# yharby/flac-raster

Hardware: AMD Instinct MI355X
Metric: raster MPixels/sec encoded at -c 5 + size ratio vs libFLAC, 1/2/4/8 GPU (higher is better)
Workload: dtype u16->i16 (int32 analysis, exact integer autocorrelation on i8 MFMA)

## Files before the change

### flac-raster_amd/csrc/fra_analyze_w.hip

```cpp
#include <type_traits>

#include "fra_device.h"

namespace fra {

namespace {

constexpr int kWChunks = kMaxBlock / kChunk;
constexpr int kWIters = kWChunks / 64;

struct WaveSmem {
  uint32_t sw[8 * kWChunks];
  double acf[3][9];
};
constexpr uint32_t kBufWords = 8 * kWChunks;

__device__ __forceinline__ int sdw(int t, int d) { return 8 * t + d; }
__device__ __forceinline__ int32_t wsample(const uint32_t* sw, int s) {
  const uint32_t v = sw[sdw(s >> 4, (s & 15) >> 1)];
  return (s & 1) ? hi16(v) : lo16(v);
}
__device__ __forceinline__ void wsync() {
  __builtin_amdgcn_wave_barrier();
  asm volatile("" ::: "memory");
}
constexpr int kWIterDw = 8 * 64;
constexpr int kWinW = 3;
__device__ __forceinline__ uint4 lds4(const uint32_t* p) { return *reinterpret_cast<const uint4*>(p); }
__device__ __forceinline__ void wread_d14(const uint32_t* sw, int lane, int j, uint32_t (&D)[14]) {
  const uint32_t* po = sw + 8 * lane + kWIterDw * j;
  const bool first = j == 0 && lane == 0;
  const uint32_t* pp = first ? po : po - 8;
  const uint4 p0 = lds4(pp), p1 = lds4(pp + 4), o0 = lds4(po), o1 = lds4(po + 4);
  D[0] = first ? 0u : p0.z; D[1] = first ? 0u : p0.w;
  D[2] = first ? 0u : p1.x; D[3] = first ? 0u : p1.y; D[4] = first ? 0u : p1.z; D[5] = first ? 0u : p1.w;
  D[6] = o0.x; D[7] = o0.y; D[8] = o0.z; D[9] = o0.w;
  D[10] = o1.x; D[11] = o1.y; D[12] = o1.z; D[13] = o1.w;
}
__device__ __forceinline__ void unpack28(const uint32_t (&D)[14], int32_t (&x)[28]) {
#pragma unroll
  for (int k = 0; k < 14; k++) {
    x[2 * k] = lo16(D[k]);
    x[2 * k + 1] = hi16(D[k]);
  }
}
__device__ __forceinline__ uint32_t group_sum32(uint32_t v, int ls) {
  if (ls > 0) v = up_add32<0>(v);
  if (ls > 1) v = up_add32<1>(v);
  if (ls > 2) v = up_add32<2>(v);
  if (ls > 3) v = up_add32<3>(v);
  if (ls > 4) v = up_add32<4>(v);
  if (ls > 5) v = up_add32<5>(v);
  return v;
}
__device__ __forceinline__ uint64_t group_sum64(uint64_t v, int ls) {
  if (ls > 0) v = up_add64<0>(v);
  if (ls > 1) v = up_add64<1>(v);
  if (ls > 2) v = up_add64<2>(v);
  if (ls > 3) v = up_add64<3>(v);
  if (ls > 4) v = up_add64<4>(v);
  if (ls > 5) v = up_add64<5>(v);
  return v;
}
__device__ __forceinline__ uint64_t group_sum_auto(uint64_t v, int ls) {
  if (__all(v < (1ull << (32 - ls)))) return group_sum32((uint32_t)v, ls);
  return group_sum64(v, ls);
}
__device__ __forceinline__ double rdlane_f64(double v, int l) {
  const uint64_t b = (uint64_t)__double_as_longlong(v);
  const uint32_t lo = (uint32_t)__builtin_amdgcn_readlane((int)(uint32_t)b, l);
  const uint32_t hi = (uint32_t)__builtin_amdgcn_readlane((int)(uint32_t)(b >> 32), l);
  return __longlong_as_double((long long)(((uint64_t)hi << 32) | lo));
}


template <int MAXLAG>
__device__ inline int levinson_keep(const double (&ac)[MAXLAG + 1], int max_order, double& e, double (&lp)[MAXLAG],
                                    int lo) {
  double lpc[MAXLAG];
#pragma unroll
  for (int j = 0; j < MAXLAG; j++) { lpc[j] = 0.0; lp[j] = 0.0; }
  e = 0.0;
  double err = ac[0];
  int result = max_order;
  bool done = false;
#pragma unroll
  for (int i = 0; i < MAXLAG; i++) {
    if (!done && i < max_order) {
      double r = -ac[i + 1];
#pragma unroll
      for (int j = 0; j < i; j++) r = r - lpc[j] * ac[i - j];
      r = r / err;
      lpc[i] = r;
#pragma unroll
      for (int j = 0; j < (i >> 1); j++) {
        const double tmp = lpc[j];
        lpc[j] = lpc[j] + r * lpc[i - 1 - j];
        lpc[i - 1 - j] = lpc[i - 1 - j] + r * tmp;
      }
      if (i & 1) lpc[i >> 1] = lpc[i >> 1] + lpc[i >> 1] * r;
      err = err * (1.0 - r * r);
      const bool mine = lo == i + 1;
#pragma unroll
      for (int j = 0; j <= i; j++) lp[j] = mine ? -lpc[j] : lp[j];
      e = (mine || (i == 0 && lo == 0)) ? err : e;
      if (!(err > 0.0)) {
        result = (err == 0.0) ? i + 1 : i;
        done = true;
      }
    }
  }
  return result;
}

__device__ __forceinline__ void fixed_guess2_w(const uint32_t (&ps)[5], int P, int lane, int& g1, int& g2,
                                               uint64_t& t1, uint64_t& t2) {
  uint64_t T[5];
  bool small = true;
  uint32_t pv[5];
#pragma unroll
  for (int k = 0; k < 5; k++) {
    pv[k] = lane < (1 << P) ? ps[k] : 0u;
    small = small && pv[k] < (1u << 25);
  }
  if (__all(small)) {
#pragma unroll
    for (int k = 0; k < 5; k++) T[k] = wave_sum32(pv[k]);
  } else {
#pragma unroll
    for (int k = 0; k < 5; k++) {
      uint64_t v = pv[k];
      v = up_add64<0>(v); v = up_add64<1>(v); v = up_add64<2>(v);
      v = up_add64<3>(v); v = up_add64<4>(v); v = up_add64<5>(v);
      T[k] = ((uint64_t)(uint32_t)__builtin_amdgcn_readlane((int)(uint32_t)(v >> 32), 63) << 32) |
             (uint32_t)__builtin_amdgcn_readlane((int)(uint32_t)v, 63);
    }
  }
  int h1 = -1, h2 = -1;
  uint64_t b1 = 0, b2 = 0;
#pragma unroll
  for (int k = 0; k < 5; k++) {
    const bool lt1 = h1 < 0 || T[k] < b1;
    const bool lt2 = !lt1 && (h2 < 0 || T[k] < b2);
    b2 = lt1 ? b1 : (lt2 ? T[k] : b2);
    h2 = lt1 ? h1 : (lt2 ? k : h2);
    b1 = lt1 ? T[k] : b1;
    h1 = lt1 ? k : h1;
  }
  g1 = __builtin_amdgcn_readfirstlane(h1);
  g2 = __builtin_amdgcn_readfirstlane(h2);
  t1 = b1;
  t2 = b2;
}

#ifndef FRA_W_ARITH
#define FRA_W_ARITH 0
#endif
struct WNorm {
  double two_mn, range, rcp;
  uint32_t flip;
};
template <typename T>
__device__ __forceinline__ int32_t wnorm(uint32_t r, const WNorm& q) {
  const int32_t v = (int32_t)((r ^ q.flip) - q.flip);
  const double t = fma((double)v, 2.0, q.two_mn);
  const double q0 = t * q.rcp;
  const double rr = fma(-q0, q.range, t);
  double u = fma(rr, q.rcp, q0);
  u = u - 1.0;
  u = u * 32767.0;
  return (int32_t)u;
}
template <typename T>
__device__ __forceinline__ void wload_lut(const void* base, const WaveDev& wd, int c,
                                          const int32_t* lut, uint32_t* sw, int lane, uint32_t& orv, int32_t& vmin,
                                          int32_t& vmax, bool stamp, const WNorm& wn) {
  constexpr int V = 8 / (int)sizeof(T);
  constexpr int NV = kMaxBlock / 64 / V;
  constexpr uint32_t step = 64 * V;
  using VT = VecT<T, V>;
  const uint32_t w = wd.width;
  const char* b0 = (const char*)((const T*)base + wd.off0 + (int64_t)c * wd.band_stride);
  const uint32_t rsb = wd.row_stride * (uint32_t)sizeof(T);
  const uint32_t qs = step / w, rs = step - qs * w, rstep = qs * rsb;
  uint32_t col = wd.col0 + (uint32_t)lane * V;
  uint32_t roff = 0;
  if (col >= w) {
    const uint32_t q = col / w;
    col -= q * w;
    roff = q * rsb;
  }
  VT x[NV];
#pragma unroll
  for (int kv = 0; kv < NV; kv++) {
    x[kv] = *(const VT*)(b0 + (roff + col * (uint32_t)sizeof(T)));
    col += rs;
    roff += rstep;
    if (col >= w) { col -= w; roff += rsb; }
  }
  if (stamp) FRA_WSTAMP_WAIT(11)
  uint32_t orp = 0;
  i16x2 pmin = {32767, 32767}, pmax = {-32768, -32768};
#pragma unroll
  for (int kv = 0; kv < NV; kv++) {
    int32_t g[V];
    const bool arith = FRA_W_ARITH == 1 || (FRA_W_ARITH == 2 && (kv & 1));
    const uint2 xw = __builtin_bit_cast(uint2, x[kv]);
#pragma unroll
    for (int e = 0; e < V; e++) {
      constexpr int EB = 8 * (int)sizeof(T);
      const uint32_t wsrc = e < V / 2 ? xw.x : xw.y;
      const uint32_t raw = (wsrc >> (EB * (e % (V / 2)))) & ((1u << EB) - 1u);
      g[e] = arith ? wnorm<T>(raw, wn) : *(const int32_t*)((const char*)lut + (raw << 2));
    }
    const int i = (lane + 64 * kv) * V;
#pragma unroll
    for (int h = 0; h < V / 4; h++) {
      const int s = i + 4 * h;
      const uint32_t p0 = __builtin_amdgcn_perm((uint32_t)g[4 * h + 1], (uint32_t)g[4 * h], 0x05040100u);
      const uint32_t p1 = __builtin_amdgcn_perm((uint32_t)g[4 * h + 3], (uint32_t)g[4 * h + 2], 0x05040100u);
      *reinterpret_cast<uint2*>(&sw[sdw(s >> 4, (s & 15) >> 1)]) = make_uint2(p0, p1);
      orp |= p0 | p1;
      const i16x2 a0 = __builtin_bit_cast(i16x2, p0), a1 = __builtin_bit_cast(i16x2, p1);
      pmin = __builtin_elementwise_min(pmin, __builtin_elementwise_min(a0, a1));
      pmax = __builtin_elementwise_max(pmax, __builtin_elementwise_max(a0, a1));
    }
  }
  orv |= (orp | (orp >> 16)) & 0xFFFFu;
  vmin = min(vmin, min((int32_t)pmin.x, (int32_t)pmin.y));
  vmax = max(vmax, max((int32_t)pmax.x, (int32_t)pmax.y));
  if (stamp) FRA_WSTAMP_WAIT(12)
}

template <int O>
__device__ __forceinline__ uint32_t lpc_abs16_w(const uint32_t (&D)[14], const int32_t* q, int sh, bool head) {
  constexpr int NP = (O + 1) / 2;
  fra_short2 Q[NP];
  q_pairs_rev<NP>(q, Q);
  uint32_t acc = 0;
#pragma unroll
  for (int jj = 0; jj < kChunk; jj++) {
    const int32_t r = sample_at(D, 12 + jj) - (pred_raw<NP>(D, 12 + jj, Q) >> sh);
    const uint32_t rb = (uint32_t)r ^ kBias;
    acc = sad_acc(rb, (jj < O && head) ? rb : kBias, acc);
  }
  return acc;
}

template <int O, bool K17>
__device__ __forceinline__ uint32_t lpc_abs16_pk(const uint32_t (&D)[14], const int32_t* q, int sh, bool head,
                                                 uint32_t (&pk)[kChunk / 2], uint32_t& um, uint32_t& hb) {
  constexpr int NP = (O + 1) / 2;
  fra_short2 Q[NP];
  q_pairs_rev<NP>(q, Q);
  uint32_t acc = 0;
  uint32_t u[kChunk];
  hb = 0;
#pragma unroll
  for (int jj = 0; jj < kChunk; jj++) {
    const int32_t r = sample_at(D, 12 + jj) - (pred_raw<NP>(D, 12 + jj, Q) >> sh);
    const uint32_t rb = (uint32_t)r ^ kBias;
    const bool warm = jj < O && head;
    acc = sad_acc(rb, warm ? rb : kBias, acc);
    u[jj] = warm ? 0u : zz32(r);
    um |= u[jj];
  }
#pragma unroll
  for (int p = 0; p < kChunk / 2; p++) pk[p] = (u[2 * p + 1] << 16) | (u[2 * p] & 0xFFFFu);
  if (K17 && __any(um > 0xFFFFu)) {
#pragma unroll
    for (int jj = 0; jj < kChunk; jj++) hb |= (u[jj] >> 16) << jj;
  }
  return acc;
}

}


template <int MAXLAG, int PCAP, bool K17>
#ifndef FRA_W_WAVES
#define FRA_W_WAVES 4
#endif
#ifndef FRA_W_ACF_ITERS
#define FRA_W_ACF_ITERS 4
#endif
#ifndef FRA_W_VGPR_FLOOR
#define FRA_W_VGPR_FLOOR 1
#endif
#ifndef FRA_W_WAVES_MAX
#define FRA_W_WAVES_MAX 8
#endif
__global__ void __launch_bounds__(64) __attribute__((amdgpu_waves_per_eu(FRA_W_WAVES, FRA_W_WAVES_MAX)))
k_analyze_w(JobArgs a, int src) {
  static_assert(MAXLAG == 8 && PCAP >= 4 && PCAP <= 6, "levels 3-6");
  __shared__ WaveSmem S;
  uint32_t* const sw = S.sw;
  const int lane = (int)threadIdx.x;
#if FRA_W_VGPR_FLOOR
  asm volatile("" ::: "v103");
#endif
  FRA_WSTAMP(0)
#ifndef FRA_W_XCD
#define FRA_W_XCD 1
#endif
  int bx = (int)blockIdx.x;
  if (FRA_W_XCD) {
    const int nx = (int)gridDim.x, n8 = nx & ~7;
    const int lin = bx + (int)blockIdx.y * nx;
    if ((nx & 7) == 0 && bx < n8) bx = (lin & 7) * (n8 >> 3) + (bx >> 3);
  }
  const int g = a.frame_base + bx;
  const int c = (int)blockIdx.y;
  const WaveDev wd = a.wave[g];
  if (c >= wd.nch) return;
  FRA_WSTAMP_WAIT(10)
  if (wd.n != kMaxBlock) return;
  constexpr int n = kMaxBlock;
  const int bps = wd.bps;
  const LevelCfg cfg = level_cfg(a.level);
  SfDesc* d = &a.sf[(size_t)g * a.cmax + c];
  uint32_t* const slot = a.tmp + ((size_t)g * a.cmax + c) * a.tmp_stride;
#ifdef FRA_WSTOP
  if (lane == 0) {
    d->type = 1; d->order = 0; d->wasted = 0; d->sbps = (uint8_t)bps; d->cval = 0; d->porder = 0;
    d->method = 0; d->precision = 0; d->shift = 0; d->bits = 8u + (uint32_t)n * (uint32_t)bps;
  }
#endif

  uint32_t orv = 0;
  int32_t vmin = INT32_MAX, vmax = INT32_MIN;
  const void* const raster = a.raster;
  const int32_t* const lut = a.lut + (int64_t)wd.stream * a.lut_stride;
  WNorm wn{};
  if (FRA_W_ARITH) {
    const NormParams np = norm_params(a.streams[wd.stream], a.norm[wd.stream]);
    wn.two_mn = -2.0 * np.mn;
    wn.range = np.range;
    wn.rcp = np.rcp;
    wn.flip = src == ST_I16 ? 0x8000u : (src == ST_I8 ? 0x80u : 0u);
  }
  auto load_samples = [&](uint32_t& ov, int32_t& mn, int32_t& mx, bool first) {
    if (src == ST_U8 || src == ST_I8) wload_lut<uint8_t>(raster, wd, c, lut, sw, lane, ov, mn, mx, first, wn);
    else wload_lut<uint16_t>(raster, wd, c, lut, sw, lane, ov, mn, mx, first, wn);
  };
  load_samples(orv, vmin, vmax, true);
  orv = wave_or32(orv);
  wsync();
  FRA_WSTAMP(1)
  vmin = (int32_t)(wave_min32((uint32_t)vmin ^ 0x80000000u) ^ 0x80000000u);
  vmax = (int32_t)(~wave_min32(~((uint32_t)vmax ^ 0x80000000u)) ^ 0x80000000u);
  FRA_WSTOP_AT(1, orv ^ (uint32_t)vmin ^ (uint32_t)vmax ^ sw[lane] ^ sw[2047 - lane])

  if (vmin == vmax) {
    if (lane == 0) {
      d->type = 0; d->order = 0; d->wasted = 0; d->sbps = (uint8_t)bps; d->cval = vmin;
      d->bits = 8u + (uint32_t)bps; d->porder = 0; d->method = 0; d->precision = 0; d->shift = 0;
      const uint64_t v = (uint64_t)(uint32_t)vmin & ((1ull << bps) - 1);
      const uint64_t blob = v << (64 - 8 - bps);
      slot[0] = (uint32_t)(blob >> 32);
      slot[1] = (uint32_t)blob;
    }
    return;
  }
  const int w = __builtin_ctz(orv);
  const int sbps = bps - w;
  auto shift_wasted = [&]() {
    for (int k = lane; k < (int)kBufWords; k += 64) {
      const uint32_t v = sw[k];
      const uint32_t lo = (uint32_t)(lo16(v) >> w) & 0xFFFFu, hi = (uint32_t)(hi16(v) >> w);
      sw[k] = lo | (hi << 16);
    }
  };
  if (w) shift_wasted();
  wsync();
  const uint32_t hdr = 8u + (uint32_t)w;
  const uint32_t verb = hdr + (uint32_t)n * (uint32_t)sbps;
  constexpr int P = PCAP;
  constexpr int gsl = 8 - P;
  const int prec = qlp_precision(bps, n);
  const int lmax = cfg.max_lpc;

  constexpr int npl = 6 - gsl;
  const int pj = lane >> npl;
  const int psrc = ((lane & ((1 << npl) - 1)) << gsl) | ((1 << gsl) - 1);
  uint32_t pfix[5] = {0, 0, 0, 0, 0};
  for (int j = 0; j < kWIters; j += 2) {
    const int t = 64 * j + lane;
    const bool head = t == 0;
    uint32_t D[14];
    wread_d14(sw, lane, j, D);
    int32_t x[28];
    unpack28(D, x);
    uint32_t v[28];
#pragma unroll
    for (int jx = 8; jx < 28; jx++) v[jx] = (uint32_t)x[jx] ^ kBias;
#pragma unroll
    for (int k = 0; k <= 4; k++) {
      if (k > 1) {
#pragma unroll
        for (int jx = 12 + kChunk - 1; jx >= 7 + k; jx--) v[jx] = xad_bias(v[jx - 1], v[jx]);
      }
      uint32_t s32 = 0;
#pragma unroll
      for (int jj = 0; jj < kChunk; jj++) {
        const uint32_t ab = v[12 + jj];
        const uint32_t bb = k == 0 ? kBias : ((jj < k && head) ? ab : v[11 + jj]);
// ... 63 lines not shown
    uint32_t p0 = lane, p1 = lane + 1, p2 = lane + 2, p3 = lane + 3;
#pragma unroll
    for (int k = 0; k < FRA_WPAD / 4; k++) {
      asm volatile("v_add_u32 %0, %0, %1" : "+v"(p0) : "v"(p1));
      asm volatile("v_add_u32 %0, %0, %1" : "+v"(p1) : "v"(p2));
      asm volatile("v_add_u32 %0, %0, %1" : "+v"(p2) : "v"(p3));
      asm volatile("v_add_u32 %0, %0, %1" : "+v"(p3) : "v"(p0));
    }
    asm volatile("" ::"v"(p0 ^ p1 ^ p2 ^ p3));
  }
#endif
  FRA_WSTAMP(3)
  FRA_WSTOP_AT(3, pf1 ^ pf2 ^ (uint32_t)(g1 * 8 + g2))
  int nlpc = 0;
  uint32_t mv = 0;
  if constexpr (MAXLAG > 0) {
    if (cfg.nsub > 0 && lmax > 0) {
      nlpc = a.nwin;
      const int nwin = a.nwin;
      constexpr int NL = MAXLAG + 1;
      double acl[NL];
      for (int wi = 0; wi < nwin; wi++) {
        const int32_t* wr = a.wrange + 2 * ((size_t)wd.win * a.nwin + wi);
        const int32_t* wp = a.wplat + 2 * ((size_t)wd.win * a.nwin + wi);
        const int lo = wr[0], hi = wr[1], plo = wp[0], phi = wp[1];
        const float* win = a.win + ((size_t)wd.win * a.nwin + wi) * a.blocksize;
        const int ri = lane & 15, g4 = lane >> 4;
        i32x4 c0h = {0, 0, 0, 0}, c0m = c0h, c0l = c0h, c1h = c0h, c1m = c0h, c1l = c0h;
        int32_t ysh = 0, ysl = 0, yfirst = 0;
        const int16_t* const sh16 = reinterpret_cast<const int16_t*>(sw);
        for (int blk = 0; blk < kWIters; blk++) {
          const int b0 = 1024 * blk;
          int sb = b0 + 256 * g4 + ri;
          asm volatile("" : "+v"(sb));
          const int16_t* const sp = sh16 + sb;
          const float* const wp = win + sb;
          const int kind = (!(lo < b0 + 1024 && hi > b0) || blk >= FRA_W_ACF_ITERS) ? 0
                           : (b0 >= plo && b0 + 1024 <= phi) ? 1 : 2;
          uint32_t H[5], L[5];
#pragma unroll
          for (int hf = 0; hf < 2; hf++) {
            int32_t y[8];
            if (kind == 0) {
#pragma unroll
              for (int e = 0; e < 8; e++) y[e] = 0;
            } else if (kind == 1) {
#pragma unroll
              for (int e = 0; e < 8; e++) y[e] = sp[16 * (8 * hf + e)];
            } else {
              float wc[8];
#pragma unroll
              for (int e = 0; e < 8; e++) wc[e] = wp[16 * (8 * hf + e)];
#pragma unroll
              for (int e = 0; e < 8; e++) y[e] = (int32_t)__builtin_rintf((float)sp[16 * (8 * hf + e)] * wc[e]);
            }
            if (blk == 0 && hf == 0) yfirst = y[0];
#pragma unroll
            for (int dd = 0; dd < 2; dd++) {
              const uint32_t p01 = __builtin_amdgcn_perm((uint32_t)y[4 * dd + 1], (uint32_t)y[4 * dd], 0x05010400u);
              const uint32_t p23 = __builtin_amdgcn_perm((uint32_t)y[4 * dd + 3], (uint32_t)y[4 * dd + 2], 0x05010400u);
              L[2 * hf + dd] = __builtin_amdgcn_perm(p23, p01, 0x05040100u) ^ 0x80808080u;
              H[2 * hf + dd] = __builtin_amdgcn_perm(p23, p01, 0x07060302u);
              ysh = __builtin_amdgcn_sdot4((int)H[2 * hf + dd], 0x01010101, ysh, false);
              ysl = __builtin_amdgcn_sdot4((int)L[2 * hf + dd], 0x01010101, ysl, false);
            }
            if (hf == 0) asm volatile("" ::: "memory");
          }
          int32_t y16;
          {
            const bool in = blk < kWIters - 1 || g4 < 3;
            const float x16 = in ? (float)sp[256] : 0.0f;
            y16 = (int32_t)__builtin_rintf(x16 * (in ? wp[256] : 0.0f));
          }
          H[4] = (uint32_t)y16 >> 8;
          L[4] = (uint32_t)y16 ^ 0x80u;
          const i32x4 xh = {(int)H[0], (int)H[1], (int)H[2], (int)H[3]};
          const i32x4 xl = {(int)L[0], (int)L[1], (int)L[2], (int)L[3]};
          const i32x4 sh = {(int)__builtin_amdgcn_alignbyte(H[1], H[0], 1), (int)__builtin_amdgcn_alignbyte(H[2], H[1], 1),
                            (int)__builtin_amdgcn_alignbyte(H[3], H[2], 1), (int)__builtin_amdgcn_alignbyte(H[4], H[3], 1)};
          const i32x4 sl = {(int)__builtin_amdgcn_alignbyte(L[1], L[0], 1), (int)__builtin_amdgcn_alignbyte(L[2], L[1], 1),
                            (int)__builtin_amdgcn_alignbyte(L[3], L[2], 1), (int)__builtin_amdgcn_alignbyte(L[4], L[3], 1)};
          c0h = __builtin_amdgcn_mfma_i32_16x16x64_i8(xh, xh, c0h, 0, 0, 0);
          c0m = __builtin_amdgcn_mfma_i32_16x16x64_i8(xh, xl, c0m, 0, 0, 0);
          c0m = __builtin_amdgcn_mfma_i32_16x16x64_i8(xl, xh, c0m, 0, 0, 0);
          c0l = __builtin_amdgcn_mfma_i32_16x16x64_i8(xl, xl, c0l, 0, 0, 0);
          c1h = __builtin_amdgcn_mfma_i32_16x16x64_i8(xh, sh, c1h, 0, 0, 0);
          c1m = __builtin_amdgcn_mfma_i32_16x16x64_i8(xh, sl, c1m, 0, 0, 0);
          c1m = __builtin_amdgcn_mfma_i32_16x16x64_i8(xl, sh, c1m, 0, 0, 0);
          c1l = __builtin_amdgcn_mfma_i32_16x16x64_i8(xl, sl, c1l, 0, 0, 0);
        }
        double mq = 0.0;
#pragma unroll
        for (int q = 0; q < 4; q++) {
          const int dd = ri - 4 * g4 - q;
          const bool in0 = dd >= 0;
          const double v = fma((double)(in0 ? c0h[q] : c1h[q]), 65536.0,
                               fma((double)(in0 ? c0m[q] : c1m[q]), 256.0, (double)(in0 ? c0l[q] : c1l[q])));
          mq = mq + __shfl(v, 16 * g4 + ((ri + 4 * g4 + q) & 15), 64);
        }
        mq = mq + __shfl_xor(mq, 16, 64);
        mq = mq + __shfl_xor(mq, 32, 64);
        const int32_t ytot = (int32_t)wave_sum32((uint32_t)(256 * ysh + ysl)) + 128 * kMaxBlock;
        int32_t pre = 0;
#pragma unroll
        for (int m = 0; m < MAXLAG; m++) {
          const int32_t vm = __builtin_amdgcn_readlane(yfirst, m);
          pre += ri > m ? vm : 0;
        }
        const double rl = mq + (256.0 * (double)ytot - 128.0 * (double)pre - 67108864.0);
        if (lane < NL) S.acf[wi][lane] = rl;
      }
      wsync();
      {
        const int gw = min(lane >> 4, nwin - 1);
#pragma unroll
        for (int l = 0; l < NL; l++) acl[l] = S.acf[gw][l];
      }
      FRA_WSTAMP(4)
#ifdef FRA_WSTOP
      {
        uint64_t kx = 0;
#pragma unroll
        for (int l = 0; l < NL; l++) kx ^= (uint64_t)__double_as_longlong(acl[l]);
        FRA_WSTOP_AT(4, kx ^ (kx >> 32))
      }
// ... 49 lines not shown
  bool kept_fit = false;
  uint64_t hk = 0;
  bool hk_any = false;
  uint32_t w4[4] = {0, 0, 0, 0};
  uint64_t lpcT = ~0ull;
#pragma unroll 1
  for (int ci = 0; ci < nlpc + 2; ci++) {
    int m, o, sh = 0, type = 2;
    int32_t qm[8] = {0, 0, 0, 0, 0, 0, 0, 0};
    uint64_t psum = 0;
    if (ci >= nlpc) {
      m = o = ci == nlpc ? g1 : g2;
      if (o < 0 || (lpcT != ~0ull && (ci == nlpc ? gt1 : gt2) >= lpcT)) continue;
      psum = ci == nlpc ? pf1 : pf2;
    } else {
      const int wi = (ci + keep_wi + 1) % nlpc;
      if (!((okm >> wi) & 1u)) continue;
      const uint32_t inf = (uint32_t)__builtin_amdgcn_readlane((int)mv, 24 + wi);
      o = (int)(inf >> 8);
      m = 5 + wi;
      type = 3;
      sh = (int)(inf & 0xFFu);
#pragma unroll
      for (int jx = 0; jx < 8; jx++) qm[jx] = __builtin_amdgcn_readlane((int)mv, 8 * wi + jx);
      if (wi == keep_wi) {
        uint32_t um = 0, carry[6] = {0, 0, 0, 0, 0, 0};
        auto keep_iter = [&](const int j, auto headc) {
          constexpr bool kHead = decltype(headc)::value;
          const bool head = kHead && lane == 0;
          uint32_t* const po = sw + 8 * lane + kWIterDw * j;
          uint32_t D[14];
          wread_d14(sw, lane, j, D);
          if (j > 0) {
#pragma unroll
            for (int k = 0; k < 6; k++) D[k] = lane == 0 ? carry[k] : D[k];
          }
#pragma unroll
          for (int k = 0; k < 6; k++) carry[k] = (uint32_t)__builtin_amdgcn_readlane((int)D[8 + k], 63);
          if (j == 0) {
#pragma unroll
            for (int k = 0; k < 4; k++) w4[k] = (uint32_t)__builtin_amdgcn_readlane((int)D[6 + k], 0);
          }
          uint32_t acc = 0, pk[kChunk / 2], hb = 0;
          switch (o) {
#define FRA_CASE(O_) \
  case O_: acc = lpc_abs16_pk<O_, K17>(D, qm, sh, head, pk, um, hb); break;
            FRA_CASE(1) FRA_CASE(2) FRA_CASE(3) FRA_CASE(4) FRA_CASE(5) FRA_CASE(6) FRA_CASE(7) FRA_CASE(8)
#undef FRA_CASE
          }
          wsync();
#pragma unroll
          for (int p = 0; p < kChunk / 4; p++) *reinterpret_cast<uint2*>(po + 2 * p) = make_uint2(pk[2 * p], pk[2 * p + 1]);
          hk |= (uint64_t)hb << (16 * j);
          const uint64_t gs = bperm64(group_sum_auto(2ull * acc, gsl), psrc);
          psum = pj == j ? gs : psum;
        };
        keep_iter(0, std::true_type{});
#pragma unroll 1
        for (int j = 1; j < kWIters; j++) keep_iter(j, std::false_type{});
        const bool need17 = __any(um > 0xFFFFu) && !__any(um > 0x1FFFFu);
        if (need17 && lane == 0 && a.cnt17) atomicAdd(a.cnt17, 1u);
        if constexpr (K17) {
          kept_fit = !__any(um > 0x1FFFFu);
          hk_any = __any(hk != 0);
        } else {
          kept_fit = !__any(um > 0xFFFFu);
        }
      } else {
#pragma unroll 1
        for (int j = 0; j < kWIters; j++) {
          const int t = 64 * j + lane;
          const bool head = t == 0;
          uint32_t D[14];
          wread_d14(sw, lane, j, D);
          uint32_t acc = 0;
          switch (o) {
#define FRA_CASE(O_) \
  case O_: acc = lpc_abs16_w<O_>(D, qm, sh, head); break;
            FRA_CASE(1) FRA_CASE(2) FRA_CASE(3) FRA_CASE(4) FRA_CASE(5) FRA_CASE(6) FRA_CASE(7) FRA_CASE(8)
#undef FRA_CASE
          }
          const uint64_t gs = bperm64(group_sum_auto(2ull * acc, gsl), psrc);
          psum = pj == j ? gs : psum;
        }
      }
      uint64_t tv = psum;
      tv = up_add64<0>(tv); tv = up_add64<1>(tv); tv = up_add64<2>(tv);
      tv = up_add64<3>(tv); tv = up_add64<4>(tv); tv = up_add64<5>(tv);
      const uint64_t T = ((uint64_t)(uint32_t)__builtin_amdgcn_readlane((int)(uint32_t)(tv >> 32), 63) << 32) |
                         (uint32_t)__builtin_amdgcn_readlane((int)(uint32_t)tv, 63);
      lpcT = T < lpcT ? T : lpcT;
    }
    constexpr int pm = P;
    uint64_t best;
    int bp;
    uint32_t kreg;
    porder_search_reg(psum, P, pm, n, o, lane, best, bp, kreg);
    const uint64_t est = hdr + (uint64_t)o * sbps + (type == 3 ? 9 + (uint64_t)o * prec : 0) + best;
    offer((uint32_t)est, m, type, o, sh, bp, kreg);
  }

  FRA_WSTAMP(6)
  FRA_WSTOP_AT(6, west ^ (uint32_t)wm ^ (uint32_t)wps)
  const int type = wtype, o = wo, sh = wsh, ps = wps;
  int32_t wq[8];
#pragma unroll
  for (int jq = 0; jq < 8; jq++) wq[jq] = type == 3 ? __builtin_amdgcn_readlane((int)mv, 8 * (wm - 5) + jq) : 0;
  const bool kept_w = type == 3 && wm == 5 + keep_wi && kept_fit;
  FRA_WSTAMP_VAL(9, kept_w ? 0 : (type != 3 ? 3 : (wm != 5 + keep_wi ? 4 : 5)))
  auto reload = [&]() {
    wsync();
    uint32_t ov = 0;
    int32_t mn = 0, mx = 0;
    load_samples(ov, mn, mx, false);
    wsync();
    if (w) shift_wasted();
    wsync();
  };
  const int pz = n >> ps;
  const int tl = 8 - ps;
  const int ls = tl < 6 ? tl : 6;
  const int npp = 1 << ps;
  auto tail = [&](auto kept_tag) {
    constexpr bool kept = decltype(kept_tag)::value;
    int32_t warm = 0;
    if (kept) {
      const uint32_t wv2 = lane >= 6 ? w4[3] : lane >= 4 ? w4[2] : lane >= 2 ? w4[1] : w4[0];
      warm = lane < o ? ((lane & 1) ? hi16(wv2) : lo16(wv2)) : 0;
    } else if (lane < o) {
      warm = wsample(sw, lane);
    }
    fra_short2 Q[4];
    q_pairs_rev<4>(wq, Q);
    auto residuals = [&](int j, uint32_t (&un)[kChunk], uint32_t (&cy)[6]) {
      const int t = 64 * j + lane;
      if (kept) {
        const uint32_t* po = sw + 8 * lane + kWIterDw * j;
#pragma unroll
        for (int p = 0; p < kChunk / 4; p++) {
          const uint2 v = *reinterpret_cast<const uint2*>(po + 2 * p);
          un[4 * p] = v.x & 0xFFFFu;
          un[4 * p + 1] = v.x >> 16;
          un[4 * p + 2] = v.y & 0xFFFFu;
          un[4 * p + 3] = v.y >> 16;
        }
        if (hk_any) {
          const uint32_t h = (uint32_t)(hk >> (16 * j));
#pragma unroll
          for (int jj = 0; jj < kChunk; jj++) un[jj] |= ((h >> jj) & 1u) << 16;
        }
        return;
      }
      uint32_t D[14];
      wread_d14(sw, lane, j, D);
      if (j > 0) {
#pragma unroll
        for (int k = 0; k < 6; k++) D[k] = lane == 0 ? cy[k] : D[k];
      }
#pragma unroll
      for (int k = 0; k < 6; k++) cy[k] = (uint32_t)__builtin_amdgcn_readlane((int)D[8 + k], 63);
      if (type == 3) {
#pragma unroll
        for (int jj = 0; jj < kChunk; jj++) un[jj] = zz32(sample_at(D, 12 + jj) - (pred_raw<4>(D, 12 + jj, Q) >> sh));
      } else {
        int32_t x[28];
        unpack28(D, x);
#pragma unroll
        for (int k = 1; k <= 4; k++) {
          if (k <= o) {
#pragma unroll
            for (int jx = 12 + kChunk - 1; jx >= 8 + k; jx--) x[jx] = x[jx] - x[jx - 1];
          }
        }
#pragma unroll
        for (int jj = 0; jj < kChunk; jj++) un[jj] = zz32(x[12 + jj]);
      }
#pragma unroll
      for (int jj = 0; jj < 12; jj++)
        if (t == 0 && jj < o) un[jj] = 0u;
    };
    uint32_t kc[kWIters];
    uint32_t fk[kWIters][3];
    uint32_t k0r[kWIters];
    uint32_t bitsl = 0;
    bool bigl = false;
    uint64_t E[3] = {0, 0, 0};
    uint32_t cyx[6] = {0, 0, 0, 0, 0, 0};
#pragma unroll
    for (int j = 0; j < kWIters; j++) {
      const int t = 64 * j + lane;
      const int pidx = t >> tl;
      const int k0 = __shfl((int)wk, pidx & 63, 64);
      const int km = k0 > 0 ? k0 - 1 : 0;
      uint32_t f0 = 0, f1 = 0, f2 = 0;
      if constexpr (kept) {
        const uint32_t* po = sw + 8 * lane + kWIterDw * j;
        typedef unsigned short u16x2 __attribute__((ext_vector_type(2)));
        auto sh = [](int k) -> u16x2 {
          const unsigned short c = (unsigned short)(k < 15 ? k : 15);
          return u16x2{c, c};
        };
        auto wt = [](int k) -> u16x2 {
          const unsigned short c = k < 16 ? 1 : 0;
          return u16x2{c, c};
        };
        const u16x2 sm = sh(km), s0 = sh(k0), s1 = sh(k0 + 1), mm = wt(km), m0 = wt(k0), m1 = wt(k0 + 1);
        if (hk_any) {
          const uint32_t c = (uint32_t)__builtin_popcount((uint32_t)(hk >> (16 * j)) & 0xFFFFu);
          f0 = km <= 16 ? c << (16 - km) : 0u;
          f1 = k0 <= 16 ? c << (16 - k0) : 0u;
          f2 = k0 + 1 <= 16 ? c << (15 - k0) : 0u;
        }
#pragma unroll
        for (int p = 0; p < kChunk / 4; p++) {
          const uint2 v = *reinterpret_cast<const uint2*>(po + 2 * p);
          const u16x2 w0 = __builtin_bit_cast(u16x2, v.x), w1 = __builtin_bit_cast(u16x2, v.y);
// ... 66 lines not shown
            const int kk = k0 + dk;
            if (kk < 0 || kk > 30) continue;
            const uint64_t e = cnt * (uint64_t)(kk + 1) + E[dk + 1];
            if (first || e < best) { best = e; bk = kk; first = false; }
          }
          if (lane == 0) {
            bitsl += (uint32_t)best;
            d->k[pq] = (uint8_t)bk;
          }
          bigl = bigl || bk > 14;
#pragma unroll
          for (int jx = 0; jx < kWIters; jx++)
            if (jx <= j && jx > j - span) kc[jx] = (uint32_t)bk;
          E[0] = E[1] = E[2] = 0;
        }
      }
    }
    FRA_WSTAMP(7)
    const bool big = __any(bigl);
    const uint64_t rtot = (uint64_t)wave_sum32(bitsl) + (uint64_t)npp * (big ? 5 : 4) + 6;
    const uint64_t exact = hdr + (uint64_t)o * sbps + (type == 3 ? 9 + (uint64_t)o * prec : 0) + rtot;
    FRA_WSTOP_AT_T(7, exact)
    const bool verbatim = exact >= verb;
    const uint32_t smask = (1u << sbps) - 1u;
    if (kept && verbatim) {
      FRA_WSTAMP_VAL(9, 6)
      return false;
    }
    if (!kept && verbatim) {
      if (lane == 0) {
        d->type = 1; d->order = 0; d->wasted = (uint8_t)w; d->sbps = (uint8_t)sbps; d->cval = 0; d->porder = 0;
        d->method = 0; d->precision = 0; d->shift = 0; d->bits = verb;
      }
      const uint32_t nwv = (verb + 31) >> 5;
      const uint64_t hv = ((uint64_t)(2u | (w ? 1u : 0u)) << 56) | (w ? (1ull << (63 - (8 + w - 1))) : 0ull);
      for (uint32_t jw = lane; jw < nwv; jw += 64) {
        const int64_t wb = 32 * (int64_t)jw;
        uint32_t word = jw == 0 ? (uint32_t)(hv >> 32) : (jw == 1 ? (uint32_t)hv : 0u);
        const int s0 = wb > (int64_t)hdr ? (int)((wb - (int64_t)hdr) / sbps) : 0;
        for (int s = s0; s < n && (int64_t)hdr + (int64_t)s * sbps < wb + 32; s++) {
          const int64_t rel = (int64_t)hdr + (int64_t)s * sbps - wb;
          const int sft = 32 - (int)rel - sbps;
          const uint64_t v = (uint64_t)((uint32_t)wsample(sw, s) & smask);
          word |= sft >= 0 ? (uint32_t)(v << sft) : (uint32_t)(v >> -sft);
        }
        slot[jw] = word;
      }
      return true;
    }
    const uint32_t fbits = (uint32_t)exact;
    const uint32_t nw = (fbits + 31) >> 5;
    const int pb = big ? 5 : 4;
    const uint32_t pos = hdr + (uint32_t)o * sbps + (type == 3 ? 9u + (uint32_t)o * prec : 0u);
    uint32_t totl[kWIters];
    uint32_t B[kWIters + 1];
    B[0] = pos + 6;
#pragma unroll
    for (int j = 0; j < kWIters; j++) {
      const int t = 64 * j + lane;
      const uint32_t kcur = kc[j], k0 = k0r[j];
      const uint32_t f = kcur + 1 == k0 ? fk[j][0] : kcur == k0 ? fk[j][1] : fk[j][2];
      const bool pstart = ((t << 4) & (pz - 1)) == 0;
      totl[j] = f + (uint32_t)(kChunk - (t == 0 ? o : 0)) * (kcur + 1u) + (pstart ? (uint32_t)pb : 0u);
      B[j + 1] = B[j] + wave_sum32(totl[j]);
    }
    bool inlds = nw + 1 <= kBufWords;
#pragma unroll
    for (int j = 0; j + 1 < kWIters; j++) inlds = inlds && (B[j + 1] - 1) / 32 + 2 <= (uint32_t)sdw(64 * (j + 1), 0);
    if (kept && !inlds) {
      FRA_WSTAMP_VAL(9, 7)
      return false;
    }
    if (lane < kMaxLpc) {
      int32_t cv = 0;
#pragma unroll
      for (int jq = 0; jq < 8; jq++) cv = lane == jq ? wq[jq] : cv;
      d->coef[lane] = type == 3 ? cv : 0;
    }
    if (lane == 0) {
      d->wasted = (uint8_t)w; d->sbps = (uint8_t)sbps; d->cval = 0;
      d->type = (uint8_t)type; d->order = (uint8_t)o; d->porder = (uint8_t)ps; d->method = big ? 1 : 0;
      d->precision = (uint8_t)(type == 3 ? prec : 0); d->shift = (int8_t)sh; d->bits = (uint32_t)exact;
    }
    auto put_header = [&](uint32_t* buf) {
      if (lane == 0) {
        lds_put(buf, 0, (uint32_t)((type == 3 ? 31 + o : 8 + o) << 1) | (w ? 1u : 0u), 8);
        if (w) lds_put(buf, 8 + (uint32_t)(w - 1), 1u, 1);
      }
      if (lane < o) lds_put(buf, hdr + (uint32_t)lane * sbps, (uint32_t)warm & smask, sbps);
      const uint32_t ph = hdr + (uint32_t)o * sbps;
      if (type == 3 && lane == 0) {
        lds_put(buf, ph, (uint32_t)(prec - 1), 4);
        lds_put(buf, ph + 4, (uint32_t)sh & 31u, 5);
      }
      if (type == 3 && lane < o) {
        int32_t cv = 0;
#pragma unroll
        for (int jq = 0; jq < 8; jq++) cv = lane == jq ? wq[jq] : cv;
        lds_put(buf, ph + 9 + (uint32_t)lane * prec, (uint32_t)cv & ((1u << prec) - 1u), prec);
      }
      if (lane == 0) lds_put(buf, pos, ((uint32_t)(big ? 1 : 0) << 4) | (uint32_t)ps, 6);
    };
    auto put_codes = [&](uint32_t* buf, int j, const uint32_t (&un)[kChunk]) {
      const int t = 64 * j + lane;
      const bool head = t == 0;
      const uint32_t kcur = kc[j], tot = totl[j];
      const bool pstart = ((t << 4) & (pz - 1)) == 0;
      uint32_t p = B[j] + wave_incl_scan32(tot) - tot;
      if (pstart) { lds_put(buf, p, kcur, pb); p += (uint32_t)pb; }
      const uint32_t sal = 31u - kcur;
#pragma unroll
      for (int jj = 0; jj < kChunk; jj++) {
        const bool skip = jj < 12 && head && jj < o;
        const uint32_t Pp = p + (un[jj] >> kcur);
        lds_put_al(buf, Pp, skip ? 0u : ((un[jj] << sal) | 0x80000000u));
        p = skip ? p : Pp + 1u + kcur;
      }
    };
    uint32_t cye[6] = {0, 0, 0, 0, 0, 0};
    if (kept || inlds) {
      uint32_t* const buf = sw;
      uint32_t Z = 0;
#pragma unroll
      for (int j = 0; j < kWIters; j++) {
        uint32_t un[kChunk];
        residuals(j, un, cye);
        wsync();
        const uint32_t Zend = j == kWIters - 1 ? nw + 1 : (B[j + 1] - 1) / 32 + 2;
        for (uint32_t jw = Z + lane; jw < Zend; jw += 64) buf[jw] = 0u;
        Z = Zend > Z ? Zend : Z;
        wsync();
        if (j == 0) put_header(buf);
        put_codes(buf, j, un);
      }
      wsync();
      for (uint32_t jw = lane; jw < nw; jw += 64) slot[jw] = buf[jw];
      FRA_WSTAMP(8)
    } else {
      for (uint32_t jw = lane; jw <= nw; jw += 64) slot[jw] = 0u;
      __threadfence();
      put_header(slot);
#pragma unroll 1
      for (int j = 0; j < kWIters; j++) {
        uint32_t un[kChunk];
        residuals(j, un, cye);
        put_codes(slot, j, un);
      }
    }
    return true;
  };
  if (!kept_w || !tail(std::true_type{})) {
    if (keep_wi >= 0) reload();
    tail(std::false_type{});
  }
}

#ifdef FRA_STAMPS
}
extern "C" __attribute__((visibility("default"))) int fra_diag_wstamps(void* host, unsigned long long bytes) {
  if (!host) {
    void* d = nullptr;
// ... 26 lines not shown
```

Baseline: 97790.

## Use dot2 inline-asm predictors, AND-based constant detection, and cheaper rounding/scan

Replaces per-sample LPC prediction with an inline-asm block computing four predictions at once using v_dot2_i32_i16 with scalar coefficient pairs. Constant-block detection switches from min/max tracking to OR/AND bit reductions. Also swaps rintf for a magic-number float add, computes the zigzag sum as su minus sign count, and reuses one inclusive scan per iteration instead of separate sum and later scan. These cut VALU work in the hot residual loops, at the cost of hand-written asm that constrains scheduling and relies on the values fitting in 16 bits.

```diff
diff --git a/flac-raster_amd/csrc/fra_analyze_w.hip b/flac-raster_amd/csrc/fra_analyze_w.hip
--- a/flac-raster_amd/csrc/fra_analyze_w.hip
+++ b/flac-raster_amd/csrc/fra_analyze_w.hip
@@ -73,6 +73,10 @@
   return __longlong_as_double((long long)(((uint64_t)hi << 32) | lo));
 }
 
+
+__device__ __forceinline__ int32_t wround16(float x, float w) {
+  return __float_as_int(__fadd_rn(__fmul_rn(x, w), 12582912.0f));
+}
 
 template <int MAXLAG>
 __device__ inline int levinson_keep(const double (&ac)[MAXLAG + 1], int max_order, double& e, double (&lp)[MAXLAG],
@@ -173,8 +177,8 @@
 }
 template <typename T>
 __device__ __forceinline__ void wload_lut(const void* base, const WaveDev& wd, int c,
-                                          const int32_t* lut, uint32_t* sw, int lane, uint32_t& orv, int32_t& vmin,
-                                          int32_t& vmax, bool stamp, const WNorm& wn) {
+                                          const int32_t* lut, uint32_t* sw, int lane, uint32_t& orv, uint32_t& anv,
+                                          bool stamp, const WNorm& wn) {
   constexpr int V = 8 / (int)sizeof(T);
   constexpr int NV = kMaxBlock / 64 / V;
   constexpr uint32_t step = 64 * V;
@@ -199,8 +203,7 @@
     if (col >= w) { col -= w; roff += rsb; }
   }
   if (stamp) FRA_WSTAMP_WAIT(11)
-  uint32_t orp = 0;
-  i16x2 pmin = {32767, 32767}, pmax = {-32768, -32768};
+  uint32_t orp = 0, anp = 0xFFFFFFFFu;
 #pragma unroll
   for (int kv = 0; kv < NV; kv++) {
     int32_t g[V];
@@ -211,7 +214,9 @@
       constexpr int EB = 8 * (int)sizeof(T);
       const uint32_t wsrc = e < V / 2 ? xw.x : xw.y;
       const uint32_t raw = (wsrc >> (EB * (e % (V / 2)))) & ((1u << EB) - 1u);
-      g[e] = arith ? wnorm<T>(raw, wn) : *(const int32_t*)((const char*)lut + (raw << 2));
+      uint32_t off = raw << 2;
+      asm("" : "+v"(off));
+      g[e] = arith ? wnorm<T>(raw, wn) : *(const int32_t*)((const char*)lut + off);
     }
     const int i = (lane + 64 * kv) * V;
 #pragma unroll
@@ -221,16 +226,62 @@
       const uint32_t p1 = __builtin_amdgcn_perm((uint32_t)g[4 * h + 3], (uint32_t)g[4 * h + 2], 0x05040100u);
       *reinterpret_cast<uint2*>(&sw[sdw(s >> 4, (s & 15) >> 1)]) = make_uint2(p0, p1);
       orp |= p0 | p1;
-      const i16x2 a0 = __builtin_bit_cast(i16x2, p0), a1 = __builtin_bit_cast(i16x2, p1);
-      pmin = __builtin_elementwise_min(pmin, __builtin_elementwise_min(a0, a1));
-      pmax = __builtin_elementwise_max(pmax, __builtin_elementwise_max(a0, a1));
+      anp &= p0 & p1;
     }
   }
   orv |= (orp | (orp >> 16)) & 0xFFFFu;
-  vmin = min(vmin, min((int32_t)pmin.x, (int32_t)pmin.y));
-  vmax = max(vmax, max((int32_t)pmax.x, (int32_t)pmax.y));
+  anv &= anp & (anp >> 16);
   if (stamp) FRA_WSTAMP_WAIT(12)
 }
+
+#define FRA_DOT4(a, b, c, d, q, c0, c1, c2, c3)                   \
+  "v_dot2_i32_i16 %[p0], %[x" #a "], %[q" #q "], " c0 "\n\t"      \
+  "v_dot2_i32_i16 %[p1], %[x" #b "], %[q" #q "], " c1 "\n\t"      \
+  "v_dot2_i32_i16 %[p2], %[x" #c "], %[q" #q "], " c2 "\n\t"      \
+  "v_dot2_i32_i16 %[p3], %[x" #d "], %[q" #q "], " c3 "\n\t"
+#define FRA_DOT4_FIRST(a, b, c, d, q) FRA_DOT4(a, b, c, d, q, "0", "0", "0", "0")
+#define FRA_DOT4_NEXT(a, b, c, d, q) FRA_DOT4(a, b, c, d, q, "%[p0]", "%[p1]", "%[p2]", "%[p3]")
+#define FRA_SHR4                              \
+  "v_ashrrev_i32 %[p0], %[sh], %[p0]\n\t"     \
+  "v_ashrrev_i32 %[p1], %[sh], %[p1]\n\t"     \
+  "v_ashrrev_i32 %[p2], %[sh], %[p2]\n\t"     \
+  "v_ashrrev_i32 %[p3], %[sh], %[p3]"
+#define FRA_P4_OUT [p0] "=&v"(p[0]), [p1] "=&v"(p[1]), [p2] "=&v"(p[2]), [p3] "=&v"(p[3])
+template <int NP>
+__device__ __forceinline__ void pred4_w(const uint32_t (&D)[14], int b, const fra_short2 (&Q)[NP], int sh,
+                                        int32_t (&p)[4]) {
+  static_assert(NP >= 1 && NP <= 4, "orders 1-8");
+  uint32_t X[2 * NP + 2];
+#pragma unroll
+  for (int k = 0; k < 2 * NP + 2; k++) X[k] = pair_at(D, b - 2 * NP + k);
+  if constexpr (NP == 1) {
+    asm(FRA_DOT4_FIRST(0, 1, 2, 3, 0) FRA_SHR4
+        : FRA_P4_OUT
+        : [sh] "s"(sh), [q0] "s"(Q[0]), [x0] "v"(X[0]), [x1] "v"(X[1]), [x2] "v"(X[2]), [x3] "v"(X[3]));
+  } else if constexpr (NP == 2) {
+    asm(FRA_DOT4_FIRST(2, 3, 4, 5, 0) FRA_DOT4_NEXT(0, 1, 2, 3, 1) FRA_SHR4
+        : FRA_P4_OUT
+        : [sh] "s"(sh), [q0] "s"(Q[0]), [q1] "s"(Q[1]), [x0] "v"(X[0]), [x1] "v"(X[1]), [x2] "v"(X[2]), [x3] "v"(X[3]),
+          [x4] "v"(X[4]), [x5] "v"(X[5]));
+  } else if constexpr (NP == 3) {
+    asm(FRA_DOT4_FIRST(4, 5, 6, 7, 0) FRA_DOT4_NEXT(2, 3, 4, 5, 1) FRA_DOT4_NEXT(0, 1, 2, 3, 2) FRA_SHR4
+        : FRA_P4_OUT
+        : [sh] "s"(sh), [q0] "s"(Q[0]), [q1] "s"(Q[1]), [q2] "s"(Q[2]), [x0] "v"(X[0]), [x1] "v"(X[1]), [x2] "v"(X[2]),
+          [x3] "v"(X[3]), [x4] "v"(X[4]), [x5] "v"(X[5]), [x6] "v"(X[6]), [x7] "v"(X[7]));
+  } else {
+    asm(FRA_DOT4_FIRST(6, 7, 8, 9, 0) FRA_DOT4_NEXT(4, 5, 6, 7, 1) FRA_DOT4_NEXT(2, 3, 4, 5, 2)
+        FRA_DOT4_NEXT(0, 1, 2, 3, 3) FRA_SHR4
+        : FRA_P4_OUT
+        : [sh] "s"(sh), [q0] "s"(Q[0]), [q1] "s"(Q[1]), [q2] "s"(Q[2]), [q3] "s"(Q[3]), [x0] "v"(X[0]), [x1] "v"(X[1]),
+          [x2] "v"(X[2]), [x3] "v"(X[3]), [x4] "v"(X[4]), [x5] "v"(X[5]), [x6] "v"(X[6]), [x7] "v"(X[7]), [x8] "v"(X[8]),
+          [x9] "v"(X[9]));
+  }
+}
+#undef FRA_P4_OUT
+#undef FRA_SHR4
+#undef FRA_DOT4_NEXT
+#undef FRA_DOT4_FIRST
+#undef FRA_DOT4
 
 template <int O>
 __device__ __forceinline__ uint32_t lpc_abs16_w(const uint32_t (&D)[14], const int32_t* q, int sh, bool head) {
@@ -239,10 +290,16 @@
   q_pairs_rev<NP>(q, Q);
   uint32_t acc = 0;
 #pragma unroll
-  for (int jj = 0; jj < kChunk; jj++) {
-    const int32_t r = sample_at(D, 12 + jj) - (pred_raw<NP>(D, 12 + jj, Q) >> sh);
-    const uint32_t rb = (uint32_t)r ^ kBias;
-    acc = sad_acc(rb, (jj < O && head) ? rb : kBias, acc);
+  for (int jb = 0; jb < kChunk; jb += 4) {
+    int32_t p[4];
+    pred4_w<NP>(D, 12 + jb, Q, sh, p);
+#pragma unroll
+    for (int i = 0; i < 4; i++) {
+      const int jj = jb + i;
+      const int32_t r = sample_at(D, 12 + jj) - p[i];
+      const uint32_t rb = (uint32_t)r ^ kBias;
+      acc = sad_acc(rb, (jj < O && head) ? rb : kBias, acc);
+    }
   }
   return acc;
 }
@@ -253,20 +310,29 @@
   constexpr int NP = (O + 1) / 2;
   fra_short2 Q[NP];
   q_pairs_rev<NP>(q, Q);
-  uint32_t acc = 0;
+  uint32_t su = 0, ss = 0;
   uint32_t u[kChunk];
   hb = 0;
 #pragma unroll
-  for (int jj = 0; jj < kChunk; jj++) {
-    const int32_t r = sample_at(D, 12 + jj) - (pred_raw<NP>(D, 12 + jj, Q) >> sh);
-    const uint32_t rb = (uint32_t)r ^ kBias;
-    const bool warm = jj < O && head;
-    acc = sad_acc(rb, warm ? rb : kBias, acc);
-    u[jj] = warm ? 0u : zz32(r);
-    um |= u[jj];
-  }
-#pragma unroll
-  for (int p = 0; p < kChunk / 2; p++) pk[p] = (u[2 * p + 1] << 16) | (u[2 * p] & 0xFFFFu);
+  for (int jb = 0; jb < kChunk; jb += 4) {
+    int32_t p[4];
+    pred4_w<NP>(D, 12 + jb, Q, sh, p);
+#pragma unroll
+    for (int i = 0; i < 4; i++) {
+      const int jj = jb + i;
+      const int32_t r = sample_at(D, 12 + jj) - p[i];
+      uint32_t sg = (uint32_t)(r >> 31);
+      asm("" : "+v"(sg));
+      const bool warm = jj < O && head;
+      u[jj] = warm ? 0u : (((uint32_t)r << 1) ^ sg);
+      su += u[jj];
+      ss += warm ? 0u : sg;
+      um |= u[jj];
+    }
+  }
+  const uint32_t acc = su - ss;
+#pragma unroll
+  for (int p = 0; p < kChunk / 2; p++) pk[p] = __builtin_amdgcn_perm(u[2 * p + 1], u[2 * p], 0x05040100u);
   if (K17 && __any(um > 0xFFFFu)) {
 #pragma unroll
     for (int jj = 0; jj < kChunk; jj++) hb |= (u[jj] >> 16) << jj;
@@ -327,8 +393,7 @@
   }
 #endif
 
-  uint32_t orv = 0;
-  int32_t vmin = INT32_MAX, vmax = INT32_MIN;
+  uint32_t orv = 0, anv = 0xFFFFu;
   const void* const raster = a.raster;
   const int32_t* const lut = a.lut + (int64_t)wd.stream * a.lut_stride;
   WNorm wn{};
@@ -339,19 +404,19 @@
     wn.rcp = np.rcp;
     wn.flip = src == ST_I16 ? 0x8000u : (src == ST_I8 ? 0x80u : 0u);
   }
-  auto load_samples = [&](uint32_t& ov, int32_t& mn, int32_t& mx, bool first) {
-    if (src == ST_U8 || src == ST_I8) wload_lut<uint8_t>(raster, wd, c, lut, sw, lane, ov, mn, mx, first, wn);
-    else wload_lut<uint16_t>(raster, wd, c, lut, sw, lane, ov, mn, mx, first, wn);
+  auto load_samples = [&](uint32_t& ov, uint32_t& an, bool first) {
+    if (src == ST_U8 || src == ST_I8) wload_lut<uint8_t>(raster, wd, c, lut, sw, lane, ov, an, first, wn);
+    else wload_lut<uint16_t>(raster, wd, c, lut, sw, lane, ov, an, first, wn);
   };
-  load_samples(orv, vmin, vmax, true);
+  load_samples(orv, anv, true);
   orv = wave_or32(orv);
   wsync();
   FRA_WSTAMP(1)
-  vmin = (int32_t)(wave_min32((uint32_t)vmin ^ 0x80000000u) ^ 0x80000000u);
-  vmax = (int32_t)(~wave_min32(~((uint32_t)vmax ^ 0x80000000u)) ^ 0x80000000u);
-  FRA_WSTOP_AT(1, orv ^ (uint32_t)vmin ^ (uint32_t)vmax ^ sw[lane] ^ sw[2047 - lane])
-
-  if (vmin == vmax) {
+  anv = ~wave_or32(~anv) & 0xFFFFu;
+  FRA_WSTOP_AT(1, orv ^ (anv << 16) ^ sw[lane] ^ sw[2047 - lane])
+
+  if (anv == orv) {
+    const int32_t vmin = lo16(orv);
     if (lane == 0) {
       d->type = 0; d->order = 0; d->wasted = 0; d->sbps = (uint8_t)bps; d->cval = vmin;
       d->bits = 8u + (uint32_t)bps; d->porder = 0; d->method = 0; d->precision = 0; d->shift = 0;
@@ -521,9 +586,9 @@
 #pragma unroll
               for (int e = 0; e < 8; e++) wc[e] = wp[16 * (8 * hf + e)];
 #pragma unroll
-              for (int e = 0; e < 8; e++) y[e] = (int32_t)__builtin_rintf((float)sp[16 * (8 * hf + e)] * wc[e]);
+              for (int e = 0; e < 8; e++) y[e] = wround16((float)sp[16 * (8 * hf + e)], wc[e]);
             }
-            if (blk == 0 && hf == 0) yfirst = y[0];
+            if (blk == 0 && hf == 0) yfirst = lo16((uint32_t)y[0]);
 #pragma unroll
             for (int dd = 0; dd < 2; dd++) {
               const uint32_t p01 = __builtin_amdgcn_perm((uint32_t)y[4 * dd + 1], (uint32_t)y[4 * dd], 0x05010400u);
@@ -539,7 +604,7 @@
           {
             const bool in = blk < kWIters - 1 || g4 < 3;
             const float x16 = in ? (float)sp[256] : 0.0f;
-            y16 = (int32_t)__builtin_rintf(x16 * (in ? wp[256] : 0.0f));
+            y16 = wround16(x16, in ? wp[256] : 0.0f);
           }
           H[4] = (uint32_t)y16 >> 8;
           L[4] = (uint32_t)y16 ^ 0x80u;
@@ -695,7 +760,7 @@
 #pragma unroll
           for (int p = 0; p < kChunk / 4; p++) *reinterpret_cast<uint2*>(po + 2 * p) = make_uint2(pk[2 * p], pk[2 * p + 1]);
           hk |= (uint64_t)hb << (16 * j);
-          const uint64_t gs = bperm64(group_sum_auto(2ull * acc, gsl), psrc);
+          const uint64_t gs = bperm64(group_sum_auto((uint64_t)acc, gsl), psrc);
           psum = pj == j ? gs : psum;
         };
         keep_iter(0, std::true_type{});
@@ -753,9 +818,8 @@
   FRA_WSTAMP_VAL(9, kept_w ? 0 : (type != 3 ? 3 : (wm != 5 + keep_wi ? 4 : 5)))
   auto reload = [&]() {
     wsync();
-    uint32_t ov = 0;
-    int32_t mn = 0, mx = 0;
-    load_samples(ov, mn, mx, false);
+    uint32_t ov = 0, an = 0;
+    load_samples(ov, an, false);
     wsync();
     if (w) shift_wasted();
     wsync();
@@ -804,7 +868,12 @@
       for (int k = 0; k < 6; k++) cy[k] = (uint32_t)__builtin_amdgcn_readlane((int)D[8 + k], 63);
       if (type == 3) {
 #pragma unroll
-        for (int jj = 0; jj < kChunk; jj++) un[jj] = zz32(sample_at(D, 12 + jj) - (pred_raw<4>(D, 12 + jj, Q) >> sh));
+        for (int jb = 0; jb < kChunk; jb += 4) {
+          int32_t p[4];
+          pred4_w<4>(D, 12 + jb, Q, sh, p);
+#pragma unroll
+          for (int i = 0; i < 4; i++) un[jb + i] = zz32(sample_at(D, 12 + jb + i) - p[i]);
+        }
       } else {
         int32_t x[28];
         unpack28(D, x);
@@ -977,7 +1046,7 @@
     const uint32_t nw = (fbits + 31) >> 5;
     const int pb = big ? 5 : 4;
     const uint32_t pos = hdr + (uint32_t)o * sbps + (type == 3 ? 9u + (uint32_t)o * prec : 0u);
-    uint32_t totl[kWIters];
+    uint32_t excl[kWIters];
     uint32_t B[kWIters + 1];
     B[0] = pos + 6;
 #pragma unroll
@@ -986,8 +1055,10 @@
       const uint32_t kcur = kc[j], k0 = k0r[j];
       const uint32_t f = kcur + 1 == k0 ? fk[j][0] : kcur == k0 ? fk[j][1] : fk[j][2];
       const bool pstart = ((t << 4) & (pz - 1)) == 0;
-      totl[j] = f + (uint32_t)(kChunk - (t == 0 ? o : 0)) * (kcur + 1u) + (pstart ? (uint32_t)pb : 0u);
-      B[j + 1] = B[j] + wave_sum32(totl[j]);
+      const uint32_t tot = f + (uint32_t)(kChunk - (t == 0 ? o : 0)) * (kcur + 1u) + (pstart ? (uint32_t)pb : 0u);
+      const uint32_t sc = wave_incl_scan32(tot);
+      excl[j] = sc - tot;
+      B[j + 1] = B[j] + (uint32_t)__builtin_amdgcn_readlane((int)sc, 63);
     }
     bool inlds = nw + 1 <= kBufWords;
 #pragma unroll
@@ -1029,9 +1100,9 @@
     auto put_codes = [&](uint32_t* buf, int j, const uint32_t (&un)[kChunk]) {
       const int t = 64 * j + lane;
       const bool head = t == 0;
-      const uint32_t kcur = kc[j], tot = totl[j];
+      const uint32_t kcur = kc[j];
       const bool pstart = ((t << 4) & (pz - 1)) == 0;
-      uint32_t p = B[j] + wave_incl_scan32(tot) - tot;
+      uint32_t p = B[j] + excl[j];
       if (pstart) { lds_put(buf, p, kcur, pb); p += (uint32_t)pb; }
       const uint32_t sal = 31u - kcur;
 #pragma unroll
```

Measured after the change: 100,100, median of 6. 2.3% higher.
